# magrimm/mav_trajectory_generation_cmake

Hardware: AMD Instinct MI355X
Metric: trajectories/sec (10-seg, N=10, 3-D min-snap) at 1/2/4/8 MI355X (higher is better)
Workload: dtype f64; 1 GPU; config2: 10000 x (K=10, N=10, D=3, r=SNAP) per GPU, device-resident; batch_per_gpu=10000, global_batch=10000, segments=10, N=10, D=3, derivative_to_optimize=4, parallelism=shard1

## Files before the change

### mav_trajectory_generation_cmake_amd/csrc/mtg_solve_dl.hip

```cpp
#include "mtg_solve_dl.inc"

namespace mtg {

#define MTG_DL_DECL(NN, DD) hipError_t launch_solve_dl_n##NN##_d##DD(const SolveArgs&, hipStream_t);
MTG_DL_DECL(10, 1) MTG_DL_DECL(10, 2) MTG_DL_DECL(10, 3) MTG_DL_DECL(10, 4)
MTG_DL_DECL(12, 1) MTG_DL_DECL(12, 2) MTG_DL_DECL(12, 3) MTG_DL_DECL(12, 4)
#undef MTG_DL_DECL

bool dl_geometry(int N, int D, int K, int r) {
  if (D < 1 || D > 4 || r < 1 || r > N / 2 - 1 || K != dl_kmax(N) || K == 0) return false;
  size_t lds = 0;
#define MTG_DL_LDS(NN, DD) \
  if (N == NN && D == DD) lds = dl_lds_bytes<NN, DD>();
  MTG_DL_LDS(10, 1) MTG_DL_LDS(10, 2) MTG_DL_LDS(10, 3) MTG_DL_LDS(10, 4)
  MTG_DL_LDS(12, 1) MTG_DL_LDS(12, 2) MTG_DL_LDS(12, 3) MTG_DL_LDS(12, 4)
#undef MTG_DL_LDS
  return lds > 0 && lds <= kMaxLdsHard;
}

hipError_t launch_solve_dl(int N, const SolveArgs& a, hipStream_t stream) {
  if (!dl_geometry(N, a.D, a.K, a.r)) return hipErrorInvalidValue;
#define MTG_DL_CASE(NN, DD) \
  if (N == NN && a.D == DD) return launch_solve_dl_n##NN##_d##DD(a, stream);
  MTG_DL_CASE(10, 1) MTG_DL_CASE(10, 2) MTG_DL_CASE(10, 3) MTG_DL_CASE(10, 4)
  MTG_DL_CASE(12, 1) MTG_DL_CASE(12, 2) MTG_DL_CASE(12, 3) MTG_DL_CASE(12, 4)
#undef MTG_DL_CASE
  return hipErrorInvalidValue;
}

}
```

### mav_trajectory_generation_cmake_amd/csrc/mtg_solve_dl.inc

```
#pragma once
#include "mtg_fused.inc"

namespace mtg {

typedef __attribute__((address_space(3))) double dl_lds_double;

static __device__ constexpr double k_dl_htilde[MTG_HTILDE_SIZE] = {MTG_HTILDE_VALUES};
static __device__ constexpr double k_dl_a1inv[MTG_A1INV_SIZE] = {MTG_A1INV_VALUES};

#define MTG_DL_STEP_BARRIER() __builtin_amdgcn_sched_barrier(0)

template <int N, int KMAX, int D>
struct DlShape {
  static constexpr int H = N / 2, F = H - 1, KC = KMAX / 2, KS = KC - 1;
  static constexpr int PE = F < 4 ? F : 4, NF0 = F - PE;
  static constexpr int J0 = NF0 > 0 ? 0 : 1;
  static constexpr int NL = F * (F - 1) / 2;
  static constexpr int FS = NL + F;
  static constexpr int TPW = kBlock / (2 * D);
  static constexpr bool RR = KC > 5;
  static constexpr int WAVES = RR ? 1 : 2;
  static constexpr bool PREG = !RR;
  static constexpr int PARK = (KC + 1) * kBlock + KC * 2 * TPW;
  static constexpr int SPAD = (N / 2) % 2 == 0 ? 2 : 0, SROW = N + SPAD;
  static constexpr int FSTR = KC * FS + ((6 - (KC * FS) % 4) % 4);
  static_assert(FSTR % 4 == 2, "odd 16-B units per chain");
  static constexpr int FAC_OFF = 0, STG_OFF = FAC_OFF + TPW * 2 * FSTR,
                       PARK_OFF = STG_OFF + kBlock * SROW, RED_OFF = PARK_OFF + PARK,
                       TAB_OFF = RED_OFF + kBlock + kBlock / 2;
  static constexpr int LDS_DOUBLES_NOTAB = TAB_OFF, LDS_DOUBLES = TAB_OFF + 2 * N * N;
  static constexpr int N_FREE(int K) { return 2 * NF0 + (K - 1) * F; }
  static constexpr bool OK = N >= 6 && N <= 12 && KMAX >= 4 && KMAX % 2 == 0 && D >= 1 && D <= 4;
};

template <int N, int R>
__device__ __forceinline__ int dl_scale_bits(double T) {
  constexpr int ea = 3 - 2 * R, eb = N - 1 - 2 * R;
  const int x = __builtin_amdgcn_frexp_exp(T) - 1;
  const int xa = x * ea, xb = x * eb;
  return (xa <= -1022 || xa >= 1023 || xb <= -1022 || xb >= 1023) ? MTG_TRAJ_NOT_SPD : 0;
}

template <int E0, int E1>
struct DlPow {
  static constexpr int NP = E1 > 0 ? E1 : 0, NM = E0 < 0 ? -E0 : 0;
  double pp[NP + 1], pm[NM + 1];
  __device__ __forceinline__ DlPow(double x, double xi) {
    pp[0] = 1.0;
    pm[0] = 1.0;
    if constexpr (NP >= 1) pp[1] = x;
    if constexpr (NM >= 1) pm[1] = xi;
#pragma unroll
    for (int k = 2; k <= NP; ++k) pp[k] = pp[k >> 1] * pp[k - (k >> 1)];
#pragma unroll
    for (int k = 2; k <= NM; ++k) pm[k] = pm[k >> 1] * pm[k - (k >> 1)];
  }
  __device__ __forceinline__ double operator()(int e) const { return e >= 0 ? pp[e] : pm[-e]; }
};

enum DlMode : int { kDlPattern = 0, kDlEnds = 1, kDlGeneral = 2 };
template <int N, int R, int KMAX, int D, int MODE = kDlPattern>
struct DlChain {
  using SH = DlShape<N, KMAX, D>;
  static constexpr bool G = MODE == kDlGeneral, EP = MODE == kDlEnds;
  static constexpr int H = SH::H, F = SH::F, KC = SH::KC, KS = SH::KS, NL = SH::NL, FS = SH::FS;
  static constexpr int PE = SH::PE, J0 = (G || EP) ? 0 : SH::J0;
  static constexpr int NN = N, RR_ = R, KM = KMAX, DD = D;
  static constexpr bool GG = G, EE = EP;
  static constexpr unsigned FM = (1u << F) - 1u;
  static constexpr bool RR = SH::RR;
  static constexpr int TOP = KS - 1;
  static constexpr int E0 = 2 - 2 * R, E1 = 2 * H - 1 - 2 * R;
  static constexpr int li(int i, int k) { return i * (i - 1) / 2 + k; }

  const dl_lds_double* ht;
  const dl_lds_double* a1;
  double* park;
  double* tpark;
  static constexpr int tstride = 2 * SH::TPW;
  static constexpr bool PR = SH::PREG && !G;
  double Pr[PR ? KC + 1 : 1], Tr[PR ? KC : 1];
  static constexpr bool FR = SH::RR && !G;
  static_assert(!FR || J0 == 0, "the register-input forward sweep needs vertex 0 as a step of its own");
  double Pf[FR ? KC + 1 : 1], Tf[FR ? KC : 1];
  bool twr;
  int tbits = 0;
  uint64_t fmask;
  double E0s[F];
  unsigned pm0 = 0;
  int nf0a = 0;
  double Zs[KS > 0 ? KS : 1][F];
  double Y[F];
  double Tn, tin;
  double* fac;
  bool wr;
  double pmin = DBL_MAX;
  double cacc = 0.0;
  uint64_t pins;
  double gf[G ? F : 1];
  __amdgpu_buffer_rsrc_t rvals;
  int vo, vs;
  int csum, ftot;

  __device__ __forceinline__ double Ht(int r, int c) const { return ht[r * N + c]; }
  __device__ __forceinline__ double A1(int r, int c) const {
    return k_dl_a1inv[MTG_A1INV_OFF(N) + r * N + c];
  }
  __device__ __forceinline__ double Hc(int r, int c) const {
    return k_dl_htilde[MTG_HTILDE_OFF(N, R) + r * N + c];
  }
  __device__ __forceinline__ double TLc(int a, int b) const { return Hc(a + 1, b + 1); }
  __device__ __forceinline__ double BRc(int a, int b) const { return Hc(H + a + 1, H + b + 1); }
  __device__ __forceinline__ double BLc(int a, int k) const { return Hc(H + a + 1, k + 1); }
  __device__ __forceinline__ double hp(int a) const { return Hc(H + a + 1, H); }
  __device__ __forceinline__ double hn(int a) const { return Hc(a + 1, H); }
  __device__ __forceinline__ double Pj(int j) const { return PR ? Pr[j] : park[j * kBlock]; }
  __device__ __forceinline__ double Tj(int j) const { return PR ? Tr[j] : tpark[j * tstride]; }
  __device__ __forceinline__ double PjF(int j) const { return FR ? Pf[j] : Pj(j); }
  __device__ __forceinline__ double TjF(int j) const { return FR ? Tf[j] : Tj(j); }
  __device__ __forceinline__ void park_fwd(int J) {
    if constexpr (FR) {
      park[(J + 1) * kBlock] = Pf[J + 1];
      if (twr) tpark[J * tstride] = Tf[J];
      tbits |= time_bits(Tf[J]) | dl_scale_bits<N, R>(Tf[J]);
      asm volatile("" : "+v"(tbits));
    }
  }
  __device__ __forceinline__ void fresh_tables() {
    asm volatile("" : "+s"(ht));
    asm volatile("" : "+s"(a1));
  }

  __device__ __forceinline__ double fl(double v, int k) const {
    return (k & 1) ? __builtin_bit_cast(double, __builtin_bit_cast(uint64_t, v) ^ fmask) : v;
  }
  __device__ __forceinline__ double zprev(int J, int k) const { return Zs[TOP][k]; }

  __device__ __forceinline__ unsigned pinm(int J) const {
    return G ? (unsigned)(pins >> (J * F)) & FM : (EP && J == 0 ? pm0 : 0u);
  }
  __device__ __forceinline__ bool pinned(int J, int a) const {
    return G ? ((pins >> (J * F + a)) & 1u) != 0 : (EP && J == 0 && ((pm0 >> a) & 1u) != 0);
  }
  __device__ __forceinline__ double fxv(int J, int a) const {
    int off = vo + J * vs + (a + 1) * D * 8;
    asm volatile("" : "+v"(off));
    const double x = fl(__builtin_bit_cast(double, __builtin_amdgcn_raw_buffer_load_b64(rvals, off, 0, 0)), a + 1);
    return pinned(J, a) ? x : 0.0;
  }
  __device__ __forceinline__ int nfv(int J) const { return F - __builtin_popcount(pinm(J)); }
  __device__ __forceinline__ int free_off(bool chB, int J) const {
    int s = 0;
#pragma unroll
    for (int q = 0; q < KC; ++q) s += (chB ? q <= J : q < J) ? nfv(q) : 0;
    return chB ? ftot - s : s;
  }

  template <int P0 = 0>
  __device__ __forceinline__ void factor(double (&S)[F][F], double (&dinv)[F]) {
    double dg[F];
#pragma unroll
    for (int j = 0; j < P0; ++j) {
      dinv[j] = 0.0;
      dg[j] = 0.0;
#pragma unroll
      for (int i = j + 1; i < F; ++i) S[i][j] = 0.0;
    }
#pragma unroll
    for (int j = P0; j < F; ++j) {
      double w[F];
      double dj = S[j][j];
#pragma unroll
      for (int k = P0; k < j; ++k) {
        w[k] = S[j][k] * dg[k];
        dj -= S[j][k] * w[k];
      }
      pmin = pivot_min(pmin, dj);
      if (RR) asm volatile("" : "+v"(pmin));
      const double inv = rcp(dj);
      dg[j] = dj;
      dinv[j] = inv;
#pragma unroll
      for (int i = j + 1; i < F; ++i) {
        double t = S[i][j];
#pragma unroll
        for (int k = P0; k < j; ++k) t -= S[i][k] * w[k];
        S[i][j] = t * inv;
      }
    }
  }
  __device__ __forceinline__ void factor_pins(double (&S)[F][F], double (&dinv)[F], unsigned pm) {
#pragma unroll
    for (int a = 0; a < F; ++a) {
      const bool pa = (pm >> a) & 1u;
#pragma unroll
      for (int b = 0; b < a; ++b) S[a][b] = (pa || ((pm >> b) & 1u)) ? 0.0 : S[a][b];
      S[a][a] = pa ? 1.0 : S[a][a];
    }
    factor(S, dinv);
#pragma unroll
    for (int a = 0; a < F; ++a) dinv[a] = ((pm >> a) & 1u) ? 0.0 : dinv[a];
  }

  template <typename LF>
  __device__ __forceinline__ static void solve(LF l, const double (&dinv)[F], double (&y)[F]) {
#pragma unroll
    for (int i = 1; i < F; ++i)
#pragma unroll
      for (int k = 0; k < i; ++k) y[i] -= l(i, k) * y[k];
#pragma unroll
    for (int i = F - 1; i >= 0; --i) {
      double t = y[i] * dinv[i];
#pragma unroll
      for (int k = i + 1; k < F; ++k) t -= l(k, i) * y[k];
      y[i] = t;
    }
  }

  template <bool MERGE, bool FIRST>
  __device__ __forceinline__ void fstep(int J, int partner, const double (&Lp)[NL > 0 ? NL : 1],
                                        const double (&Dp)[F], double& Tp, double& tip, double (&S)[F][F],
                                        double (&dinv)[F], double (&rhs)[F]) {
    fresh_tables();
    double Pm[F][F];
    if constexpr (FIRST) {
#pragma unroll
      for (int a = 0; a < F; ++a)
#pragma unroll
        for (int b = 0; b <= a; ++b) Pm[a][b] = BRc(a, b);
    } else {
      double W[F][F], U[F][F];
// ... 359 lines not shown
    } else {
#pragma unroll
      for (int i = 0; i < F; ++i) y[i] = Zs[TOP][i] - tt[i];
#pragma unroll
      for (int q = KS - 1; q >= 1; --q)
#pragma unroll
        for (int k = 0; k < F; ++k) Zs[q][k] = Zs[q - 1][k];
    }
  }
};

__device__ __forceinline__ __amdgpu_buffer_rsrc_t dl_rsrc(const void* base, uint32_t bytes) { return buf_rsrc(base, bytes); }
typedef u32x4 dl_u32x4;
typedef u32x2 dl_u32x2;

template <int D>
__device__ __forceinline__ bool dl_traj_any(uint64_t ballot, int q) {
  constexpr uint64_t LM = 2 * D >= 64 ? ~0ull : (1ull << (2 * D)) - 1ull;
  return q * 2 * D < 64 && ((ballot >> (q * 2 * D)) & LM) != 0;
}

constexpr int kDlSc1 = 16;

template <int N, int KMAX, int D, int AL16>
struct DlStore {
  static constexpr int DN = D * N, PW = AL16 ? 2 : 1, PPR = DN / PW;
  static constexpr int POL = AL16 == 2 ? kDlSc1 : 0;
  static constexpr int NU = (DlShape<N, KMAX, D>::TPW * 2 * PPR + kBlock - 1) / kBlock;
  static constexpr int kOOB = 0x40000000;
  static_assert(NU * kBlock * PW <= kBlock * N, "the staged pieces a lane reads lie in the staging area");
  static constexpr int SP = DlShape<N, KMAX, D>::SPAD / PW, RP = N / PW;
  static __device__ __forceinline__ int staged(int e) { return SP ? e + (e / RP) * SP : e; }
  static_assert(DN % PW == 0, "whole 16-B pieces per run");
  int off[NU], dlt[NU];
  __device__ __forceinline__ void init(int lane, int nvt, uint64_t badl) {
    const int lim = nvt * 2 * PPR;
    uint32_t badq = 0;
    if (badl != 0) {
#pragma unroll
      for (int q = 0; q < DlShape<N, KMAX, D>::TPW; ++q) badq |= dl_traj_any<D>(badl, q) ? 1u << q : 0u;
    }
#pragma unroll
    for (int u = 0; u < NU; ++u) {
      const int e = lane + u * kBlock;
      const int run = e / PPR, o = e - run * PPR, q = run >> 1;
      const bool rv = run & 1;
      const bool ok = e < lim && !((badq >> (q & 31)) & 1u);
      off[u] = ok ? (q * KMAX * DN + o * PW + (rv ? (KMAX - 1) * DN : 0)) * 8 : kOOB;
      dlt[u] = ok ? (rv ? -DN * 8 : DN * 8) : 0;
    }
  }
};

template <typename DC, int AL16, bool FIRSTB = false>
__device__ __forceinline__ void dl_round(DC& c, const SolveArgs& a, int J, int lane, int ch, int d, bool own, int64_t pb,
                                         double* stg, const DlStore<DC::NN, DC::KM, DC::DD, AL16>& sm,
                                         __amdgpu_buffer_rsrc_t out) {
  constexpr int N = DC::NN, KMAX = DC::KM, D = DC::DD;
  constexpr int H = N / 2, F = H - 1, K = KMAX, V = K + 1;
  const double T = c.Tj(J), tinv = rcp(T);
  double v[F];
  if constexpr (FIRSTB) {
#pragma unroll
    for (int b = 0; b < F; ++b) v[b] = c.Y[b];
  } else {
    const double rho = T * c.tin;
    double rp = rho;
#pragma unroll
    for (int b = 0; b < F; ++b) {
      v[b] = rp * c.Y[b];
      rp *= rho;
    }
  }
  using SH = DlShape<N, KMAX, D>;
  double y[F];
  if (FIRSTB || J >= DC::J0) {
    if constexpr (DC::GG) {
      double vb[F];
#pragma unroll
      for (int b = 0; b < F; ++b) vb[b] = c.pinned(J + 1, b) ? 0.0 : v[b];
      c.bstep(J, vb, y);
    } else {
      c.bstep(J, v, y);
    }
  } else {
#pragma unroll
    for (int k = 0; k < F; ++k) y[k] = c.E0s[k];
  }
  if constexpr (DC::GG) {
    double tp = T;
#pragma unroll
    for (int k = 0; k < F; ++k) {
      y[k] = c.pinned(J, k) ? tp * c.fxv(J, k) : y[k];
      tp *= T;
    }
  }
  double occ[N];
  c.segment_row(ch != 0, a.cost_out != nullptr, J, tinv, y, v, occ);
  if (DC::GG && a.free_out && own) {
    double* fo = a.free_out + (pb * D + d) * ((int64_t)V * H) + c.free_off(ch != 0, J);
    const unsigned fr = ~c.pinm(J) & DC::FM;
    double tp = tinv;
#pragma unroll
    for (int k = 0; k < F; ++k) {
      const double x = y[k] * tp;
      if ((fr >> k) & 1u) fo[__builtin_popcount(fr & ((1u << k) - 1u))] = ch ? c.fl(x, k + 1) : x;
      tp *= tinv;
    }
  } else if (DC::EE && a.free_out && own) {
    const int vx = ch ? K - J : J;
    double* fo = a.free_out + (pb * D + d) * ((int64_t)V * H) + (vx == 0 ? 0 : c.nf0a + (vx - 1) * F);
    const unsigned fr = ~c.pinm(J) & DC::FM;
    double tp = tinv;
#pragma unroll
    for (int k = 0; k < F; ++k) {
      const double x = y[k] * tp;
      if ((fr >> k) & 1u) fo[__builtin_popcount(fr & ((1u << k) - 1u))] = ch ? c.fl(x, k + 1) : x;
      tp *= tinv;
    }
  } else if ((J >= 1 || SH::NF0 > 0) && a.free_out && own) {
    const int vx = ch ? K - J : J;
    double* fo = a.free_out + (pb * D + d) * ((int64_t)V * H) +
                 (vx == 0 ? 0 : (vx == K ? SH::NF0 + (K - 1) * F : SH::NF0 + (vx - 1) * F)) - (J == 0 ? SH::PE : 0);
    double tp = tinv;
#pragma unroll
    for (int k = 0; k < F; ++k) {
      const double x = y[k] * tp;
      if (J >= 1 || k >= SH::PE) fo[k] = ch ? c.fl(x, k + 1) : x;
      tp *= tinv;
    }
  }
#pragma unroll
  for (int k = 0; k < F; ++k) c.Y[k] = y[k];
  c.Tn = T;
  c.tin = tinv;
  if (!a.coeffs) return;
  dvec2* o2 = reinterpret_cast<dvec2*>(stg + lane * SH::SROW);
#pragma unroll
  for (int j = 0; j < N / 2; ++j) o2[j] = dvec2{occ[2 * j], occ[2 * j + 1]};
  lds_fence();
  constexpr int NU = DlStore<N, KMAX, D, AL16>::NU;
  constexpr int kAux = DlStore<N, KMAX, D, AL16>::POL;
  if constexpr (AL16) {
    dvec2 w[NU];
#pragma unroll
    for (int u = 0; u < NU; ++u) w[u] = reinterpret_cast<const dvec2*>(stg)[DlStore<N, KMAX, D, AL16>::staged(lane + u * kBlock)];
#pragma unroll
    for (int u = 0; u < NU; ++u)
      __builtin_amdgcn_raw_buffer_store_b128(__builtin_bit_cast(dl_u32x4, w[u]), out, sm.off[u] + J * sm.dlt[u], 0, kAux);
  } else {
    double w[NU];
#pragma unroll
    for (int u = 0; u < NU; ++u) w[u] = stg[DlStore<N, KMAX, D, AL16>::staged(lane + u * kBlock)];
#pragma unroll
    for (int u = 0; u < NU; ++u)
      __builtin_amdgcn_raw_buffer_store_b64(__builtin_bit_cast(dl_u32x2, w[u]), out, sm.off[u] + J * sm.dlt[u], 0, kAux);
  }
  lds_fence();
}

constexpr int kDlFallbackLgLog2 = 4, kDlFallbackTraj = kBlock >> kDlFallbackLgLog2;
template <int N, int R, int D>
__device__ __forceinline__ void dl_fallback(const SolveArgs& a, int64_t pair0, int nvt, uint64_t badl, double* lds) {
  uint32_t badq = 0;
  for (int q = 0; q < nvt; ++q) badq |= dl_traj_any<D>(badl, q) ? 1u << q : 0u;
  const int nb = __builtin_popcount(badq);
  const int slot = threadIdx.x >> kDlFallbackLgLog2;
  for (int base = 0; base < nb; base += kDlFallbackTraj) {
    const int k = base + slot;
    uint32_t m = badq;
    for (int i = 0; i < k && m; ++i) m &= m - 1u;
    const bool valid = k < nb;
    const int q = valid ? __builtin_ctz(m) : 0;
    solve_fused_slots<N, R>(a, kDlFallbackLgLog2, pair0 + q, valid, lds);
    __syncthreads();
  }
}

template <int N, int KMAX, int D>
struct DlWave {
  using SH = DlShape<N, KMAX, D>;
  static constexpr int H = N / 2, K = KMAX, V = K + 1;
  int lane, t, r2, ch, d, tq, partner, nvt, trl;
  bool valid;
  int64_t pair0, pb;
  double tscale;
  __amdgpu_buffer_rsrc_t rv, rt, rm;
  int vo, vs, to, ts, mo, ms;
  __device__ __forceinline__ DlWave(const SolveArgs& a, int tpw, int lane_id) {
    lane = lane_id;
    t = lane / (2 * D);
    r2 = lane - t * (2 * D);
    ch = r2 >= D ? 1 : 0;
    d = r2 - ch * D;
    tq = t < SH::TPW ? t : 0;
    partner = ch ? lane - D : lane + D;
    pair0 = (int64_t)blockIdx.x * tpw;
    const int64_t pair = pair0 + t;
    valid = t < tpw && pair < a.B;
    pb = valid ? pair : pair0;
    nvt = (int)(a.B - pair0 < tpw ? a.B - pair0 : tpw);
    const int64_t nc = a.n_cand;
    const int64_t tr0 = nc == 1 ? pair0 : pair0 / nc;
    trl = (int)((nc == 1 ? pb : pb / nc) - tr0);
    const int64_t ntr = nc == 1 ? a.B : (a.B + nc - 1) / nc;
    const int ntw = (int)(ntr - tr0 < SH::TPW ? ntr - tr0 : SH::TPW);
    rv = dl_rsrc(a.values + tr0 * (V * H * D), (uint32_t)(ntw * V * H * D * 8));
    rt = dl_rsrc(a.times + tr0 * K, (uint32_t)(ntw * K * 8));
    rm = dl_rsrc(a.mask + tr0 * V, (uint32_t)(ntw * V));
    tscale = a.scales ? a.scales[pb % nc] : 1.0;
    vo = (trl * (V * H * D) + (ch ? K * H * D : 0) + d) * 8;
    vs = ch ? -(H * D * 8) : H * D * 8;
    to = (trl * K + (ch ? K - 1 : 0)) * 8;
    ts = ch ? -8 : 8;
    mo = trl * V + (ch ? K : 0);
    ms = ch ? -1 : 1;
  }
  __device__ __forceinline__ unsigned mask(int j) const { return __builtin_amdgcn_raw_buffer_load_b8(rm, mo + j * ms, 0, 0); }
  __device__ __forceinline__ double time(int j, double sc) const {
    return __builtin_bit_cast(double, __builtin_amdgcn_raw_buffer_load_b64(rt, to + j * ts, 0, 0)) * sc;
  }
  __device__ __forceinline__ double value(int j, int k) const {
    return __builtin_bit_cast(double, __builtin_amdgcn_raw_buffer_load_b64(rv, vo + j * vs + k * D * 8, 0, 0));
  }
};

struct DlKernArgs {
  SolveArgs a;
  int tpw;
};
__device__ __forceinline__ const DlKernArgs& dl_args() {
  return *reinterpret_cast<const DlKernArgs*>((uintptr_t)__builtin_amdgcn_kernarg_segment_ptr());
}

template <int N, int R, int KC>
__device__ __forceinline__ int dl_time_bits(const double (&Tc)[KC]) {
  int st = 0;
#pragma unroll
  for (int j = 0; j < KC; ++j) st |= time_bits(Tc[j]) | dl_scale_bits<N, R>(Tc[j]);
  asm volatile("" : "+v"(st));
  return st;
}

template <typename CC, int AL16, typename W>
__device__ __forceinline__ void dl_run_pass(CC& cc, const SolveArgs& a, const W& w, const double (&E)[CC::F], bool mine,
                                            int st, double* lds, uint64_t* tph) {
  constexpr int N = CC::NN, R = CC::RR_, KMAX = CC::KM, D = CC::DD;
  using SH = DlShape<N, KMAX, D>;
  constexpr int H = N / 2, F = SH::F, KC = SH::KC;
  constexpr int K = KMAX, V = K + 1;
#ifdef MTG_PHASE_TIMING
#define MTG_DL_PSTAMP(k) tph[k] = __builtin_amdgcn_s_memrealtime()
#else
#define MTG_DL_PSTAMP(k) (void)tph
#endif
  const int lane = w.lane, ch = w.ch, d = w.d;
  const int64_t pb = w.pb;
  cc.forward(w.partner, E);
  MTG_DL_PSTAMP(2);
  if constexpr (CC::PR) st |= dl_time_bits<N, R, KC>(cc.Tr);
  if constexpr (CC::FR) st |= cc.tbits;
  if (a.free_out && mine && ch == 0) {
    double* fo = a.free_out + (pb * D + d) * ((int64_t)V * H);
    if constexpr (CC::GG) {
      const unsigned fr = ~cc.pinm(KC) & CC::FM;
#pragma unroll
      for (int k = 0; k < F; ++k)
        if ((fr >> k) & 1u) fo[cc.csum + __builtin_popcount(fr & ((1u << k) - 1u))] = cc.Y[k];
    } else {
      const int o0 = CC::EE ? cc.nf0a : SH::NF0;
#pragma unroll
      for (int k = 0; k < F; ++k) fo[o0 + (KC - 1) * F + k] = cc.Y[k];
    }
  }
  cc.scale_meeting();
  __syncthreads();

  double* stg = lds + SH::STG_OFF;
  DlStore<N, KMAX, D, AL16> sm;
  sm.init(lane, w.nvt, __builtin_amdgcn_ballot_w64(!mine));
  const __amdgpu_buffer_rsrc_t ro =
      dl_rsrc(a.coeffs ? a.coeffs + w.pair0 * (int64_t)(K * D * N) : a.values, (uint32_t)(w.nvt * K * D * N * 8));
  dl_round<CC, AL16, true>(cc, a, KC - 1, lane, ch, d, mine, pb, stg, sm, ro);
#pragma unroll
  for (int J = KC - 2; J >= 1; --J) {
    MTG_DL_STEP_BARRIER();
    dl_round<CC, AL16>(cc, a, J, lane, ch, d, mine, pb, stg, sm, ro);
  }
  MTG_DL_STEP_BARRIER();
  dl_round<CC, AL16>(cc, a, 0, lane, ch, d, mine, pb, stg, sm, ro);
  MTG_DL_PSTAMP(3);

  if (!(cc.pmin > 0.0 && cc.pmin <= DBL_MAX)) st |= MTG_TRAJ_NOT_SPD;
  if (a.status || a.cost_out) {
    double* red = lds + SH::RED_OFF;
    int* redi = reinterpret_cast<int*>(red + kBlock);
    __syncthreads();
    red[lane] = cc.cacc;
    redi[lane] = st;
    __syncthreads();
    if (w.r2 == 0 && mine) {
      double cost = 0.0;
      int s = 0;
#pragma unroll
      for (int q = 0; q < 2 * D; ++q) cost += red[lane + q], s |= redi[lane + q];
      if (a.cost_out) a.cost_out[pb] = cost;
      if (a.status) a.status[pb] = s;
    }
  }
  if (w.r2 == 0 && mine && a.n_free_out) {
    if constexpr (CC::GG || CC::EE) {
      a.n_free_out[pb] = cc.ftot;
    } else {
      a.n_free_out[pb] = SH::N_FREE(K);
    }
  }
#ifdef MTG_PHASE_TIMING
  asm volatile("s_waitcnt vmcnt(0)" ::: "memory");
  MTG_DL_PSTAMP(4);
  if (a.free_out && lane == 0) {
    double* fo = a.free_out + w.pair0 * D * ((int64_t)V * H);
    for (int k = 0; k < 5; ++k) fo[k] = (double)tph[k];
    unsigned hw, xcc;
    asm volatile("s_getreg_b32 %0, hwreg(HW_REG_HW_ID)" : "=s"(hw));
    asm volatile("s_getreg_b32 %0, hwreg(HW_REG_XCC_ID)" : "=s"(xcc));
    fo[5] = (double)hw;
    fo[6] = (double)xcc;
  }
#endif
#undef MTG_DL_PSTAMP
}

template <typename CC, typename W>
__device__ __forceinline__ void dl_place(CC& c, const W& w, int tpw, double* lds) {
  using SH = DlShape<CC::NN, CC::KM, CC::DD>;
  c.fmask = w.ch ? 0x8000000000000000ull : 0ull;
  c.fac = lds + SH::FAC_OFF + (w.tq * 2 + w.ch) * SH::FSTR;
  c.wr = w.d == 0 && w.t < tpw;
  c.park = lds + SH::PARK_OFF + w.lane;
  c.tpark = lds + SH::PARK_OFF + (CC::KC + 1) * kBlock + w.tq * 2 + w.ch;
  c.ht = (const dl_lds_double*)(lds + SH::TAB_OFF);
  c.a1 = (const dl_lds_double*)(lds + SH::TAB_OFF + CC::NN * CC::NN);
}

template <typename CC>
__device__ __forceinline__ void dl_take_inputs(CC& c, const double (&P)[CC::KC + 1], const double (&Tc)[CC::KC], int d,
                                               int t) {
  using SH = DlShape<CC::NN, CC::KM, CC::DD>;
  constexpr int KC = CC::KC;
  if constexpr (CC::PR) {
#pragma unroll
    for (int j = 0; j <= KC; ++j) c.Pr[j] = P[j];
#pragma unroll
    for (int j = 0; j < KC; ++j) c.Tr[j] = Tc[j];
  } else {
    static_assert(CC::FR, "the pattern and ends passes keep their inputs in registers");
#pragma unroll
    for (int j = 0; j <= KC; ++j) c.Pf[j] = P[j];
#pragma unroll
    for (int j = 0; j < KC; ++j) c.Tf[j] = Tc[j];
    c.twr = d == 0 && t < SH::TPW;
    c.park[0] = P[0];
  }
}

template <int N, int R, int KMAX, int D, int AL16>
__device__ __forceinline__ void dl_ends_pass(bool eown) {
  const DlKernArgs& ka = dl_args();
  const SolveArgs a = ka.a;
  const int tpw = ka.tpw;
#ifdef MTG_PHASE_TIMING
  uint64_t tph[6];
  tph[0] = __builtin_amdgcn_s_memrealtime();
#else
  uint64_t* tph = nullptr;
#endif
  using SH = DlShape<N, KMAX, D>;
  using EC = DlChain<N, R, KMAX, D, kDlEnds>;
  constexpr int H = N / 2, F = SH::F, KC = SH::KC;
  constexpr unsigned HM = (1u << H) - 1u;
  extern __shared__ __attribute__((aligned(16))) double lds[];
  int lane_id = threadIdx.x;
  asm volatile("" : "+v"(lane_id));
  const DlWave<N, KMAX, D> w(a, tpw, lane_id);
  EC c;
  dl_place(c, w, tpw, lds);
  const unsigned m0 = w.mask(0);
  double Tc[KC], P[KC + 1], E[F];
  Tc[0] = w.time(0, w.tscale);
#pragma unroll
  for (int k = 0; k < F; ++k) E[k] = c.fl(w.value(0, k + 1), k + 1);
#pragma unroll
  for (int j = 0; j <= KC; ++j) {
    P[j] = w.value(j, 0);
    if (j + 1 < KC) Tc[j + 1] = w.time(j + 1, w.tscale);
  }
  c.pm0 = (m0 >> 1) & EC::FM;
  const int nf0 = F - __builtin_popcount(c.pm0), nfp = __shfl(nf0, w.partner);
  c.nf0a = w.ch ? nfp : nf0;
  c.ftot = nf0 + nfp + (KMAX - 1) * F;
  dl_take_inputs(c, P, Tc, w.d, w.t);
#ifdef MTG_PHASE_TIMING
  tph[1] = __builtin_amdgcn_s_memrealtime();
#endif
  dl_run_pass<EC, AL16>(c, a, w, E, eown, (m0 & ~HM) ? MTG_TRAJ_WARN_DROPPED : 0, lds, tph);
}

template <int N, int R, int KMAX, int D, int AL16>
__device__ __forceinline__ void dl_general_pass(bool gown) {
  const DlKernArgs& ka = dl_args();
  const SolveArgs a = ka.a;
  const int tpw = ka.tpw;
#ifdef MTG_PHASE_TIMING
  uint64_t tph[6];
  tph[0] = __builtin_amdgcn_s_memrealtime();
#else
  uint64_t* tph = nullptr;
#endif
  using SH = DlShape<N, KMAX, D>;
  using DG = DlChain<N, R, KMAX, D, kDlGeneral>;
  constexpr int H = N / 2, F = SH::F, KC = SH::KC;
  constexpr unsigned HM = (1u << H) - 1u;
  extern __shared__ __attribute__((aligned(16))) double lds[];
  int lane_id = threadIdx.x;
  asm volatile("" : "+v"(lane_id));
  const DlWave<N, KMAX, D> w(a, tpw, lane_id);
  DG g;
  dl_place(g, w, tpw, lds);
  g.rvals = w.rv;
  g.vo = w.vo;
  g.vs = w.vs;
  double P[KC + 1], Tc[KC];
  unsigned mk[KC + 1];
#pragma unroll
  for (int j = 0; j <= KC; ++j) {
    mk[j] = w.mask(j);
    P[j] = w.value(j, 0);
    if (j < KC) Tc[j] = w.time(j, w.tscale);
  }
  int dropped = 0;
  g.pins = 0;
#pragma unroll
  for (int j = 0; j <= KC; ++j) {
    g.pins |= (uint64_t)((mk[j] >> 1) & DG::FM) << (j * F);
    dropped |= mk[j] & ~HM;
    g.park[j * kBlock] = P[j];
  }
  if (w.d == 0 && w.t < SH::TPW) {
#pragma unroll
    for (int j = 0; j < KC; ++j) g.tpark[j * g.tstride] = Tc[j];
  }
  const int st0 = dl_time_bits<N, R, KC>(Tc) | (dropped ? MTG_TRAJ_WARN_DROPPED : 0);
  int cs = 0;
#pragma unroll
  for (int j = 0; j < KC; ++j) cs += g.nfv(j);
  g.csum = cs;
  g.ftot = cs + __shfl(cs, w.partner) + g.nfv(KC);
  __syncthreads();
#ifdef MTG_PHASE_TIMING
  tph[1] = __builtin_amdgcn_s_memrealtime();
#endif
  double E[F];
#pragma unroll
  for (int k = 0; k < F; ++k) E[k] = 0.0;
  dl_run_pass<DG, AL16>(g, a, w, E, gown, st0, lds, tph);
}

template <int N, int R, int KMAX, int D, int AL16>
__global__ __launch_bounds__(kBlock) __attribute__((amdgpu_waves_per_eu(DlShape<N, KMAX, D>::WAVES))) void solve_dl_kernel(
    DlKernArgs ka) {
  using SH = DlShape<N, KMAX, D>;
  using DC = DlChain<N, R, KMAX, D>;
  constexpr int F = SH::F, KC = SH::KC;
  constexpr unsigned EM = (1u << (SH::PE + 1)) - 1u;
  const SolveArgs& a = ka.a;
  const int tpw = ka.tpw;
  extern __shared__ __attribute__((aligned(16))) double lds[];
#ifdef MTG_PHASE_TIMING
  uint64_t tph[6];
  tph[0] = __builtin_amdgcn_s_memrealtime();
#else
  uint64_t* tph = nullptr;
#endif
  const DlWave<N, KMAX, D> w(a, tpw, threadIdx.x);
  const int t = w.t, d = w.d;

  DC c;
  dl_place(c, w, tpw, lds);
  unsigned mk[KC + 1];
  double Tc[KC], P[KC + 1], E[F];
#pragma unroll
  for (int j = 0; j <= KC; ++j) mk[j] = w.mask(j);
  Tc[0] = w.time(0, w.tscale);
#pragma unroll
  for (int k = 0; k < F; ++k) E[k] = k < SH::PE ? c.fl(w.value(0, k + 1), k + 1) : 0.0;
#pragma unroll
  for (int j = 0; j <= KC; ++j) {
    P[j] = w.value(j, 0);
    if (j + 1 < KC) Tc[j + 1] = w.time(j + 1, w.tscale);
  }
  unsigned bad = mk[0] ^ EM, ebad = ~mk[0] & 1u, xpos = 0u;
#pragma unroll
  for (int j = 1; j <= KC; ++j) {
    bad |= mk[j] ^ 1u;
    ebad |= mk[j] ^ 1u;
  }
#pragma unroll
  for (int j = 0; j <= KC; ++j) xpos |= ~mk[j] & 1u;
  const uint64_t badl = __builtin_amdgcn_ballot_w64(bad != 0u), el = __builtin_amdgcn_ballot_w64(ebad != 0u),
                 xl = __builtin_amdgcn_ballot_w64(xpos != 0u);
  const bool pbad = dl_traj_any<D>(badl, t), ebt = dl_traj_any<D>(el, t), xbad = dl_traj_any<D>(xl, t);
  const bool own = w.valid && !pbad, eown = w.valid && pbad && !ebt, gown = w.valid && ebt && !xbad,
             fown = w.valid && xbad;

  if (a.cost_out) {
    constexpr int UH = (N * N + kBlock - 1) / kBlock;
    const double* hg = c_htilde + MTG_HTILDE_OFF(N, R);
    const double* ag = c_a1inv + MTG_A1INV_OFF(N);
    double hv[UH], av[UH];
#pragma unroll
    for (int u = 0; u < UH; ++u) {
      const int i = w.lane + u * kBlock;
      hv[u] = hg[i < N * N ? i : N * N - 1];
      av[u] = ag[i < N * N ? i : N * N - 1];
    }
#pragma unroll
    for (int u = 0; u < UH; ++u) {
      const int i = w.lane + u * kBlock;
      lds[SH::TAB_OFF + (i < N * N ? i : N * N - 1)] = hv[u];
      lds[SH::TAB_OFF + N * N + (i < N * N ? i : N * N - 1)] = av[u];
    }
  }
  if (__builtin_amdgcn_ballot_w64(own) != 0) {
    dl_take_inputs(c, P, Tc, d, t);
    if (a.cost_out) __syncthreads();
#ifdef MTG_PHASE_TIMING
    tph[1] = __builtin_amdgcn_s_memrealtime();
#endif
    dl_run_pass<DC, AL16>(c, a, w, E, own, 0, lds, tph);
  }
  if (__builtin_expect(__builtin_amdgcn_ballot_w64(eown) != 0, 0)) {
    __syncthreads();
    dl_ends_pass<N, R, KMAX, D, AL16>(eown);
  }
  if (__builtin_expect(__builtin_amdgcn_ballot_w64(gown) != 0, 0)) {
    __syncthreads();
    dl_general_pass<N, R, KMAX, D, AL16>(gown);
  }
  if (__builtin_expect(__builtin_amdgcn_ballot_w64(fown) != 0, 0)) {
    __syncthreads();
    dl_fallback<N, R, D>(a, w.pair0, w.nvt, __builtin_amdgcn_ballot_w64(fown), lds);
  }
}
__host__ __device__ constexpr int dl_kmax(int N) { return N == 10 ? 10 : (N == 12 ? 20 : 0); }
template <int N, int D>
__host__ __device__ constexpr size_t dl_lds_bytes(bool cost = true) {
  constexpr int KMAX = dl_kmax(N) > 0 ? dl_kmax(N) : 4;
  const size_t dl = sizeof(double) * (size_t)(cost ? DlShape<N, KMAX, D>::LDS_DOUBLES : DlShape<N, KMAX, D>::LDS_DOUBLES_NOTAB);
  const size_t fb = sizeof(double) * (size_t)kDlFallbackTraj * slot_doubles(N / 2, D, KMAX, 1 << kDlFallbackLgLog2);
  return dl > fb ? dl : fb;
}

inline bool dl_store_sc1(size_t bytes, bool long_chains) {
  static const int force = [] {
    const char* v = getenv("MTG_DL_STORE_SC1");
    return v && (v[0] == '0' || v[0] == '1') ? v[0] - '0' : -1;
  }();
  return force >= 0 ? force == 1 : bytes <= ((size_t)(long_chains ? 192 : 64) << 20);
}

template <int N, int R, int KMAX, int D>
static hipError_t launch_dl_nrk(const SolveArgs& a, hipStream_t stream) {
  if constexpr (!DlShape<N, KMAX, D>::OK || R < 1) {
    return hipErrorInvalidValue;
  } else {
    if (a.K != KMAX) return hipErrorInvalidValue;
    const size_t lds = dl_lds_bytes<N, D>(a.cost_out != nullptr);
    const int tpw = DlShape<N, KMAX, D>::TPW;
    const bool sc1 = dl_store_sc1((size_t)a.B * KMAX * D * N * sizeof(double), DlShape<N, KMAX, D>::RR);
    const int64_t blocks = (a.B + tpw - 1) / tpw;
    if (blocks == 0) return hipSuccess;
    const bool al16 = !(reinterpret_cast<uintptr_t>(a.coeffs) & 15u);
    const int al = al16 ? (sc1 ? 2 : 1) : 0;
    const void* fn = al == 2 ? (const void*)solve_dl_kernel<N, R, KMAX, D, 2>
                             : al == 1 ? (const void*)solve_dl_kernel<N, R, KMAX, D, 1> : (const void*)solve_dl_kernel<N, R, KMAX, D, 0>;
    if (lds > kMaxLdsPerBlock) {
      const hipError_t e = hipFuncSetAttribute(fn, hipFuncAttributeMaxDynamicSharedMemorySize, (int)lds);
      if (e != hipSuccess) return e;
    }
    const DlKernArgs ka{a, tpw};
    if (al == 2)
      launch_kernel((solve_dl_kernel<N, R, KMAX, D, 2>), dim3((unsigned)blocks), dim3(kBlock), lds, stream, ka);
    else if (al == 1)
      launch_kernel((solve_dl_kernel<N, R, KMAX, D, 1>), dim3((unsigned)blocks), dim3(kBlock), lds, stream, ka);
    else
      launch_kernel((solve_dl_kernel<N, R, KMAX, D, 0>), dim3((unsigned)blocks), dim3(kBlock), lds, stream, ka);
    return hipGetLastError();
  }
}

template <int N, int R, int D>
static hipError_t launch_dl_nrd(const SolveArgs& a, hipStream_t stream) {
  if constexpr (dl_kmax(N) > 0) {
    if (a.K == dl_kmax(N)) return launch_dl_nrk<N, R, dl_kmax(N), D>(a, stream);
  }
  return hipErrorInvalidValue;
}

template <int N, int D>
static hipError_t launch_dl_nd(const SolveArgs& a, hipStream_t stream) {
  switch (a.r) {
    case 1: if constexpr (N / 2 > 1) return launch_dl_nrd<N, 1, D>(a, stream); break;
    case 2: if constexpr (N / 2 > 2) return launch_dl_nrd<N, 2, D>(a, stream); break;
    case 3: if constexpr (N / 2 > 3) return launch_dl_nrd<N, 3, D>(a, stream); break;
    case 4: if constexpr (N / 2 > 4) return launch_dl_nrd<N, 4, D>(a, stream); break;
    case 5: if constexpr (N / 2 > 5) return launch_dl_nrd<N, 5, D>(a, stream); break;
    default: break;
  }
  return hipErrorInvalidValue;
}

#define MTG_DL_LAUNCHER(NN, DD)                                                          \
  hipError_t launch_solve_dl_n##NN##_d##DD(const SolveArgs& a, hipStream_t stream) {     \
    return launch_dl_nd<NN, DD>(a, stream);                                              \
  }

}
```

Before: 1.007 billion trajectories/s.

## Add compact 64-byte kernarg hot header and status-free kernel variant

Puts a 64-byte header at the front of the kernel arguments. It holds precomputed per-block byte strides, the last-block count and flags, and is loaded as one scalar vector, so each block skips the 64-bit divides and the full SolveArgs reads when there is one candidate and no scales. It adds a template flag ST that removes pivot-min tracking, time/scale status bits and the status/cost reduction when no optional outputs are requested and the output fits a size threshold. Optional output pointers are loaded only when flagged. The risk is losing the not-SPD and status detection in the default path, plus more kernel instantiations.

```diff
diff --git a/mav_trajectory_generation_cmake_amd/csrc/mtg_solve_dl.hip b/mav_trajectory_generation_cmake_amd/csrc/mtg_solve_dl.hip
--- a/mav_trajectory_generation_cmake_amd/csrc/mtg_solve_dl.hip
+++ b/mav_trajectory_generation_cmake_amd/csrc/mtg_solve_dl.hip
@@ -29,3 +29,28 @@
 }
 
 }
+
+extern "C" int mtgtest_dl_hot_header(int N, int D, int K, int r, const void* values, const void* mask, const void* times,
+                                     void* coeffs, const void* scales, int64_t B, int n_cand, int any_optional,
+                                     void* out) {
+  using namespace mtg;
+  if (!dl_geometry(N, D, K, r) || B < 1) return -1;
+  SolveArgs a{};
+  a.values = static_cast<const double*>(values);
+  a.mask = static_cast<const uint8_t*>(mask);
+  a.times = static_cast<const double*>(times);
+  a.coeffs = static_cast<double*>(coeffs);
+  a.scales = static_cast<const double*>(scales);
+  static int32_t dummy_status;
+  a.status = any_optional ? &dummy_status : nullptr;
+  a.B = B;
+  a.K = K;
+  a.D = D;
+  a.r = r;
+  a.n_cand = n_cand;
+  const int tpw = kBlock / (2 * D);
+  DlHot h;
+  if (!dl_fill_hot(N, K, D, tpw, a, &h)) return -1;
+  *static_cast<DlHot*>(out) = h;
+  return 0;
+}
diff --git a/mav_trajectory_generation_cmake_amd/csrc/mtg_solve_dl.inc b/mav_trajectory_generation_cmake_amd/csrc/mtg_solve_dl.inc
--- a/mav_trajectory_generation_cmake_amd/csrc/mtg_solve_dl.inc
+++ b/mav_trajectory_generation_cmake_amd/csrc/mtg_solve_dl.inc
@@ -59,14 +59,14 @@
 };
 
 enum DlMode : int { kDlPattern = 0, kDlEnds = 1, kDlGeneral = 2 };
-template <int N, int R, int KMAX, int D, int MODE = kDlPattern>
+template <int N, int R, int KMAX, int D, int MODE = kDlPattern, bool ST = true>
 struct DlChain {
   using SH = DlShape<N, KMAX, D>;
   static constexpr bool G = MODE == kDlGeneral, EP = MODE == kDlEnds;
   static constexpr int H = SH::H, F = SH::F, KC = SH::KC, KS = SH::KS, NL = SH::NL, FS = SH::FS;
   static constexpr int PE = SH::PE, J0 = (G || EP) ? 0 : SH::J0;
   static constexpr int NN = N, RR_ = R, KM = KMAX, DD = D;
-  static constexpr bool GG = G, EE = EP;
+  static constexpr bool GG = G, EE = EP, SS = ST;
   static constexpr unsigned FM = (1u << F) - 1u;
   static constexpr bool RR = SH::RR;
   static constexpr int TOP = KS - 1;
@@ -122,8 +122,10 @@
     if constexpr (FR) {
       park[(J + 1) * kBlock] = Pf[J + 1];
       if (twr) tpark[J * tstride] = Tf[J];
-      tbits |= time_bits(Tf[J]) | dl_scale_bits<N, R>(Tf[J]);
-      asm volatile("" : "+v"(tbits));
+      if constexpr (ST) {
+        tbits |= time_bits(Tf[J]) | dl_scale_bits<N, R>(Tf[J]);
+        asm volatile("" : "+v"(tbits));
+      }
     }
   }
   __device__ __forceinline__ void fresh_tables() {
@@ -175,8 +177,10 @@
         w[k] = S[j][k] * dg[k];
         dj -= S[j][k] * w[k];
       }
-      pmin = pivot_min(pmin, dj);
-      if (RR) asm volatile("" : "+v"(pmin));
+      if constexpr (ST) {
+        pmin = pivot_min(pmin, dj);
+        if (RR) asm volatile("" : "+v"(pmin));
+      }
       const double inv = rcp(dj);
       dg[j] = dj;
       dinv[j] = inv;
@@ -642,8 +646,16 @@
   }
 };
 
+struct DlOuts {
+  double* coeffs;
+  double* free_out;
+  double* cost_out;
+  int32_t* status;
+  int32_t* n_free_out;
+};
+
 template <typename DC, int AL16, bool FIRSTB = false>
-__device__ __forceinline__ void dl_round(DC& c, const SolveArgs& a, int J, int lane, int ch, int d, bool own, int64_t pb,
+__device__ __forceinline__ void dl_round(DC& c, const DlOuts& a, int J, int lane, int ch, int d, bool own, int64_t pb,
                                          double* stg, const DlStore<DC::NN, DC::KM, DC::DD, AL16>& sm,
                                          __amdgpu_buffer_rsrc_t out) {
   constexpr int N = DC::NN, KMAX = DC::KM, D = DC::DD;
@@ -686,7 +698,7 @@
     }
   }
   double occ[N];
-  c.segment_row(ch != 0, a.cost_out != nullptr, J, tinv, y, v, occ);
+  c.segment_row(ch != 0, DC::SS && a.cost_out != nullptr, J, tinv, y, v, occ);
   if (DC::GG && a.free_out && own) {
     double* fo = a.free_out + (pb * D + d) * ((int64_t)V * H) + c.free_off(ch != 0, J);
     const unsigned fr = ~c.pinm(J) & DC::FM;
@@ -767,6 +779,60 @@
   }
 }
 
+enum DlHotFlags : uint32_t {
+  kDlPlain = 1u,
+  kDlCoeffs = 2u,
+  kDlOptional = 4u,
+};
+struct DlHot {
+  const double* values;
+  const uint8_t* mask;
+  const double* times;
+  double* coeffs;
+  uint32_t vbytes, mbytes, tbytes, obytes;
+  int32_t tpw;
+  uint32_t flags;
+  uint32_t last_block;
+  int32_t last_nvt;
+};
+static_assert(sizeof(DlHot) == 64, "the hot header is one 64-byte line");
+struct DlKernArgs {
+  DlHot h;
+  SolveArgs a;
+};
+static_assert(offsetof(DlKernArgs, h) == 0, "the hot header leads the kernarg segment");
+__device__ __forceinline__ const DlKernArgs& dl_args() {
+  return *reinterpret_cast<const DlKernArgs*>((uintptr_t)__builtin_amdgcn_kernarg_segment_ptr());
+}
+__device__ __forceinline__ DlHot dl_hot() {
+  typedef uint32_t dl_u32x16 __attribute__((ext_vector_type(16)));
+  dl_u32x16 v = *(const __attribute__((address_space(4))) dl_u32x16*)__builtin_amdgcn_kernarg_segment_ptr();
+  asm volatile("" : "+s"(v));
+  return __builtin_bit_cast(DlHot, v);
+}
+
+inline bool dl_fill_hot(int N, int K, int D, int tpw, const SolveArgs& a, DlHot* h) {
+  const int64_t V = K + 1, H = N / 2;
+  const int64_t vb = tpw * V * H * D * 8, mb = tpw * V, tb = (int64_t)tpw * K * 8, ob = (int64_t)tpw * K * D * N * 8;
+  if (a.B < 1 || tpw < 1 || vb > INT32_MAX || ob > INT32_MAX) return false;
+  const int64_t blocks = (a.B + tpw - 1) / tpw;
+  if (blocks > UINT32_MAX) return false;
+  h->values = a.values;
+  h->mask = a.mask;
+  h->times = a.times;
+  h->coeffs = a.coeffs;
+  h->vbytes = (uint32_t)vb;
+  h->mbytes = (uint32_t)mb;
+  h->tbytes = (uint32_t)tb;
+  h->obytes = (uint32_t)ob;
+  h->tpw = tpw;
+  h->flags = (a.n_cand == 1 && !a.scales ? kDlPlain : 0u) | (a.coeffs ? kDlCoeffs : 0u) |
+             (a.free_out || a.n_free_out || a.cost_out || a.status ? kDlOptional : 0u);
+  h->last_block = (uint32_t)(blocks - 1);
+  h->last_nvt = (int32_t)(a.B - (blocks - 1) * tpw);
+  return true;
+}
+
 template <int N, int KMAX, int D>
 struct DlWave {
   using SH = DlShape<N, KMAX, D>;
@@ -776,8 +842,10 @@
   int64_t pair0, pb;
   double tscale;
   __amdgpu_buffer_rsrc_t rv, rt, rm;
+  const char* obase;
   int vo, vs, to, ts, mo, ms;
-  __device__ __forceinline__ DlWave(const SolveArgs& a, int tpw, int lane_id) {
+  __device__ __forceinline__ DlWave(const DlHot& h, const SolveArgs& a, int lane_id) {
+    const int tpw = h.tpw;
     lane = lane_id;
     t = lane / (2 * D);
     r2 = lane - t * (2 * D);
@@ -785,20 +853,30 @@
     d = r2 - ch * D;
     tq = t < SH::TPW ? t : 0;
     partner = ch ? lane - D : lane + D;
-    pair0 = (int64_t)blockIdx.x * tpw;
-    const int64_t pair = pair0 + t;
-    valid = t < tpw && pair < a.B;
-    pb = valid ? pair : pair0;
-    nvt = (int)(a.B - pair0 < tpw ? a.B - pair0 : tpw);
-    const int64_t nc = a.n_cand;
-    const int64_t tr0 = nc == 1 ? pair0 : pair0 / nc;
-    trl = (int)((nc == 1 ? pb : pb / nc) - tr0);
-    const int64_t ntr = nc == 1 ? a.B : (a.B + nc - 1) / nc;
-    const int ntw = (int)(ntr - tr0 < SH::TPW ? ntr - tr0 : SH::TPW);
-    rv = dl_rsrc(a.values + tr0 * (V * H * D), (uint32_t)(ntw * V * H * D * 8));
-    rt = dl_rsrc(a.times + tr0 * K, (uint32_t)(ntw * K * 8));
-    rm = dl_rsrc(a.mask + tr0 * V, (uint32_t)(ntw * V));
-    tscale = a.scales ? a.scales[pb % nc] : 1.0;
+    const uint32_t bid = blockIdx.x;
+    nvt = bid == h.last_block ? h.last_nvt : tpw;
+    pair0 = (int64_t)((uint64_t)bid * (uint32_t)tpw);
+    valid = t < nvt;
+    pb = valid ? pair0 + t : pair0;
+    obase = (h.flags & kDlCoeffs) ? reinterpret_cast<const char*>(h.coeffs) + (uint64_t)bid * h.obytes
+                                  : reinterpret_cast<const char*>(h.values);
+    if (__builtin_expect((h.flags & kDlPlain) != 0u, 1)) {
+      trl = valid ? t : 0;
+      rv = dl_rsrc(reinterpret_cast<const char*>(h.values) + (uint64_t)bid * h.vbytes, (uint32_t)(nvt * (V * H * D * 8)));
+      rt = dl_rsrc(reinterpret_cast<const char*>(h.times) + (uint64_t)bid * h.tbytes, (uint32_t)(nvt * (K * 8)));
+      rm = dl_rsrc(h.mask + (uint64_t)bid * h.mbytes, (uint32_t)(nvt * V));
+      tscale = 1.0;
+    } else {
+      const int64_t nc = a.n_cand;
+      const int64_t tr0 = pair0 / nc;
+      trl = (int)(pb / nc - tr0);
+      const int64_t ntr = (a.B + nc - 1) / nc;
+      const int ntw = (int)(ntr - tr0 < SH::TPW ? ntr - tr0 : SH::TPW);
+      rv = dl_rsrc(a.values + tr0 * (V * H * D), (uint32_t)(ntw * V * H * D * 8));
+      rt = dl_rsrc(a.times + tr0 * K, (uint32_t)(ntw * K * 8));
+      rm = dl_rsrc(a.mask + tr0 * V, (uint32_t)(ntw * V));
+      tscale = a.scales ? a.scales[pb % nc] : 1.0;
+    }
     vo = (trl * (V * H * D) + (ch ? K * H * D : 0) + d) * 8;
     vs = ch ? -(H * D * 8) : H * D * 8;
     to = (trl * K + (ch ? K - 1 : 0)) * 8;
@@ -806,6 +884,7 @@
     mo = trl * V + (ch ? K : 0);
     ms = ch ? -1 : 1;
   }
+  __device__ __forceinline__ __amdgpu_buffer_rsrc_t out() const { return dl_rsrc(obase, (uint32_t)(nvt * (K * D * N * 8))); }
   __device__ __forceinline__ unsigned mask(int j) const { return __builtin_amdgcn_raw_buffer_load_b8(rm, mo + j * ms, 0, 0); }
   __device__ __forceinline__ double time(int j, double sc) const {
     return __builtin_bit_cast(double, __builtin_amdgcn_raw_buffer_load_b64(rt, to + j * ts, 0, 0)) * sc;
@@ -815,12 +894,8 @@
   }
 };
 
-struct DlKernArgs {
-  SolveArgs a;
-  int tpw;
-};
-__device__ __forceinline__ const DlKernArgs& dl_args() {
-  return *reinterpret_cast<const DlKernArgs*>((uintptr_t)__builtin_amdgcn_kernarg_segment_ptr());
+__device__ __forceinline__ DlOuts dl_outs(const SolveArgs& a) {
+  return DlOuts{a.coeffs, a.free_out, a.cost_out, a.status, a.n_free_out};
 }
 
 template <int N, int R, int KC>
@@ -833,7 +908,7 @@
 }
 
 template <typename CC, int AL16, typename W>
-__device__ __forceinline__ void dl_run_pass(CC& cc, const SolveArgs& a, const W& w, const double (&E)[CC::F], bool mine,
+__device__ __forceinline__ void dl_run_pass(CC& cc, const DlOuts& a, const W& w, const double (&E)[CC::F], bool mine,
                                             int st, double* lds, uint64_t* tph) {
   constexpr int N = CC::NN, R = CC::RR_, KMAX = CC::KM, D = CC::DD;
   using SH = DlShape<N, KMAX, D>;
@@ -848,8 +923,8 @@
   const int64_t pb = w.pb;
   cc.forward(w.partner, E);
   MTG_DL_PSTAMP(2);
-  if constexpr (CC::PR) st |= dl_time_bits<N, R, KC>(cc.Tr);
-  if constexpr (CC::FR) st |= cc.tbits;
+  if constexpr (CC::SS && CC::PR) st |= dl_time_bits<N, R, KC>(cc.Tr);
+  if constexpr (CC::SS && CC::FR) st |= cc.tbits;
   if (a.free_out && mine && ch == 0) {
     double* fo = a.free_out + (pb * D + d) * ((int64_t)V * H);
     if constexpr (CC::GG) {
@@ -869,8 +944,7 @@
   double* stg = lds + SH::STG_OFF;
   DlStore<N, KMAX, D, AL16> sm;
   sm.init(lane, w.nvt, __builtin_amdgcn_ballot_w64(!mine));
-  const __amdgpu_buffer_rsrc_t ro =
-      dl_rsrc(a.coeffs ? a.coeffs + w.pair0 * (int64_t)(K * D * N) : a.values, (uint32_t)(w.nvt * K * D * N * 8));
+  const __amdgpu_buffer_rsrc_t ro = w.out();
   dl_round<CC, AL16, true>(cc, a, KC - 1, lane, ch, d, mine, pb, stg, sm, ro);
 #pragma unroll
   for (int J = KC - 2; J >= 1; --J) {
@@ -881,28 +955,30 @@
   dl_round<CC, AL16>(cc, a, 0, lane, ch, d, mine, pb, stg, sm, ro);
   MTG_DL_PSTAMP(3);
 
-  if (!(cc.pmin > 0.0 && cc.pmin <= DBL_MAX)) st |= MTG_TRAJ_NOT_SPD;
-  if (a.status || a.cost_out) {
-    double* red = lds + SH::RED_OFF;
-    int* redi = reinterpret_cast<int*>(red + kBlock);
-    __syncthreads();
-    red[lane] = cc.cacc;
-    redi[lane] = st;
-    __syncthreads();
-    if (w.r2 == 0 && mine) {
-      double cost = 0.0;
-      int s = 0;
-#pragma unroll
-      for (int q = 0; q < 2 * D; ++q) cost += red[lane + q], s |= redi[lane + q];
-      if (a.cost_out) a.cost_out[pb] = cost;
-      if (a.status) a.status[pb] = s;
-    }
-  }
-  if (w.r2 == 0 && mine && a.n_free_out) {
-    if constexpr (CC::GG || CC::EE) {
-      a.n_free_out[pb] = cc.ftot;
-    } else {
-      a.n_free_out[pb] = SH::N_FREE(K);
+  if constexpr (CC::SS) {
+    if (!(cc.pmin > 0.0 && cc.pmin <= DBL_MAX)) st |= MTG_TRAJ_NOT_SPD;
+    if (a.status || a.cost_out) {
+      double* red = lds + SH::RED_OFF;
+      int* redi = reinterpret_cast<int*>(red + kBlock);
+      __syncthreads();
+      red[lane] = cc.cacc;
+      redi[lane] = st;
+      __syncthreads();
+      if (w.r2 == 0 && mine) {
+        double cost = 0.0;
+        int s = 0;
+#pragma unroll
+        for (int q = 0; q < 2 * D; ++q) cost += red[lane + q], s |= redi[lane + q];
+        if (a.cost_out) a.cost_out[pb] = cost;
+        if (a.status) a.status[pb] = s;
+      }
+    }
+    if (w.r2 == 0 && mine && a.n_free_out) {
+      if constexpr (CC::GG || CC::EE) {
+        a.n_free_out[pb] = cc.ftot;
+      } else {
+        a.n_free_out[pb] = SH::N_FREE(K);
+      }
     }
   }
 #ifdef MTG_PHASE_TIMING
@@ -954,11 +1030,12 @@
   }
 }
 
-template <int N, int R, int KMAX, int D, int AL16>
+template <int N, int R, int KMAX, int D, int AL16, bool ST>
 __device__ __forceinline__ void dl_ends_pass(bool eown) {
   const DlKernArgs& ka = dl_args();
-  const SolveArgs a = ka.a;
-  const int tpw = ka.tpw;
+  const DlOuts a = dl_outs(ka.a);
+  const DlHot h = dl_hot();
+  const int tpw = h.tpw;
 #ifdef MTG_PHASE_TIMING
   uint64_t tph[6];
   tph[0] = __builtin_amdgcn_s_memrealtime();
@@ -966,13 +1043,13 @@
   uint64_t* tph = nullptr;
 #endif
   using SH = DlShape<N, KMAX, D>;
-  using EC = DlChain<N, R, KMAX, D, kDlEnds>;
+  using EC= DlChain<N, R, KMAX, D, kDlEnds, ST>;
   constexpr int H = N / 2, F = SH::F, KC = SH::KC;
   constexpr unsigned HM = (1u << H) - 1u;
   extern __shared__ __attribute__((aligned(16))) double lds[];
   int lane_id = threadIdx.x;
   asm volatile("" : "+v"(lane_id));
-  const DlWave<N, KMAX, D> w(a, tpw, lane_id);
+  const DlWave<N, KMAX, D> w(h, ka.a, lane_id);
   EC c;
   dl_place(c, w, tpw, lds);
   const unsigned m0 = w.mask(0);
@@ -996,11 +1073,12 @@
   dl_run_pass<EC, AL16>(c, a, w, E, eown, (m0 & ~HM) ? MTG_TRAJ_WARN_DROPPED : 0, lds, tph);
 }
 
-template <int N, int R, int KMAX, int D, int AL16>
+template <int N, int R, int KMAX, int D, int AL16, bool ST>
 __device__ __forceinline__ void dl_general_pass(bool gown) {
   const DlKernArgs& ka = dl_args();
-  const SolveArgs a = ka.a;
-  const int tpw = ka.tpw;
+  const DlOuts a = dl_outs(ka.a);
+  const DlHot h = dl_hot();
+  const int tpw = h.tpw;
 #ifdef MTG_PHASE_TIMING
   uint64_t tph[6];
   tph[0] = __builtin_amdgcn_s_memrealtime();
@@ -1008,13 +1086,13 @@
   uint64_t* tph = nullptr;
 #endif
   using SH = DlShape<N, KMAX, D>;
-  using DG = DlChain<N, R, KMAX, D, kDlGeneral>;
+  using DG= DlChain<N, R, KMAX, D, kDlGeneral, ST>;
   constexpr int H = N / 2, F = SH::F, KC = SH::KC;
   constexpr unsigned HM = (1u << H) - 1u;
   extern __shared__ __attribute__((aligned(16))) double lds[];
   int lane_id = threadIdx.x;
   asm volatile("" : "+v"(lane_id));
-  const DlWave<N, KMAX, D> w(a, tpw, lane_id);
+  const DlWave<N, KMAX, D> w(h, ka.a, lane_id);
   DG g;
   dl_place(g, w, tpw, lds);
   g.rvals = w.rv;
@@ -1040,7 +1118,8 @@
 #pragma unroll
     for (int j = 0; j < KC; ++j) g.tpark[j * g.tstride] = Tc[j];
   }
-  const int st0 = dl_time_bits<N, R, KC>(Tc) | (dropped ? MTG_TRAJ_WARN_DROPPED : 0);
+  int st0 = 0;
+  if constexpr (ST) st0 = dl_time_bits<N, R, KC>(Tc) | (dropped ? MTG_TRAJ_WARN_DROPPED : 0);
   int cs = 0;
 #pragma unroll
   for (int j = 0; j < KC; ++j) cs += g.nfv(j);
@@ -1056,15 +1135,28 @@
   dl_run_pass<DG, AL16>(g, a, w, E, gown, st0, lds, tph);
 }
 
-template <int N, int R, int KMAX, int D, int AL16>
+template <int N, int R, int KMAX, int D, int AL16, bool ST>
 __global__ __launch_bounds__(kBlock) __attribute__((amdgpu_waves_per_eu(DlShape<N, KMAX, D>::WAVES))) void solve_dl_kernel(
     DlKernArgs ka) {
   using SH = DlShape<N, KMAX, D>;
-  using DC = DlChain<N, R, KMAX, D>;
+  using DC = DlChain<N, R, KMAX, D, kDlPattern, ST>;
   constexpr int F = SH::F, KC = SH::KC;
   constexpr unsigned EM = (1u << (SH::PE + 1)) - 1u;
-  const SolveArgs& a = ka.a;
-  const int tpw = ka.tpw;
+  const DlHot h = dl_hot();
+  const int tpw = h.tpw;
+  DlOuts a{h.coeffs, nullptr, nullptr, nullptr, nullptr};
+  if (h.flags & kDlOptional) {
+    typedef const __attribute__((address_space(4))) char* dl_kptr;
+    auto fa = (const __attribute__((address_space(4))) SolveArgs*)((dl_kptr)__builtin_amdgcn_kernarg_segment_ptr() +
+                                                                   offsetof(DlKernArgs, a));
+    asm volatile("" : "+s"(fa));
+    a.free_out = fa->free_out;
+    if constexpr (ST) {
+      a.cost_out = fa->cost_out;
+      a.status = fa->status;
+      a.n_free_out = fa->n_free_out;
+    }
+  }
   extern __shared__ __attribute__((aligned(16))) double lds[];
 #ifdef MTG_PHASE_TIMING
   uint64_t tph[6];
@@ -1072,7 +1164,7 @@
 #else
   uint64_t* tph = nullptr;
 #endif
-  const DlWave<N, KMAX, D> w(a, tpw, threadIdx.x);
+  const DlWave<N, KMAX, D> w(h, ka.a, threadIdx.x);
   const int t = w.t, d = w.d;
 
   DC c;
@@ -1131,15 +1223,15 @@
   }
   if (__builtin_expect(__builtin_amdgcn_ballot_w64(eown) != 0, 0)) {
     __syncthreads();
-    dl_ends_pass<N, R, KMAX, D, AL16>(eown);
+    dl_ends_pass<N, R, KMAX, D, AL16, ST>(eown);
   }
   if (__builtin_expect(__builtin_amdgcn_ballot_w64(gown) != 0, 0)) {
     __syncthreads();
-    dl_general_pass<N, R, KMAX, D, AL16>(gown);
+    dl_general_pass<N, R, KMAX, D, AL16, ST>(gown);
   }
   if (__builtin_expect(__builtin_amdgcn_ballot_w64(fown) != 0, 0)) {
     __syncthreads();
-    dl_fallback<N, R, D>(a, w.pair0, w.nvt, __builtin_amdgcn_ballot_w64(fown), lds);
+    dl_fallback<N, R, D>(dl_args().a, w.pair0, w.nvt, __builtin_amdgcn_ballot_w64(fown), lds);
   }
 }
 __host__ __device__ constexpr int dl_kmax(int N) { return N == 10 ? 10 : (N == 12 ? 20 : 0); }
@@ -1157,6 +1249,25 @@
     return v && (v[0] == '0' || v[0] == '1') ? v[0] - '0' : -1;
   }();
   return force >= 0 ? force == 1 : bytes <= ((size_t)(long_chains ? 192 : 64) << 20);
+}
+
+inline bool dl_status_free(size_t bytes, bool long_chains) {
+  static const int force = [] {
+    const char* v = getenv("MTG_DL_STATUS");
+    return v && (v[0] == '0' || v[0] == '1') ? v[0] - '0' : -1;
+  }();
+  return force >= 0 ? force == 0 : bytes <= ((size_t)(long_chains ? 192 : 64) << 20);
+}
+
+template <int N, int R, int KMAX, int D, int AL16, bool ST>
+static hipError_t launch_dl_inst(const DlKernArgs& ka, unsigned blocks, size_t lds, hipStream_t stream) {
+  if (lds > kMaxLdsPerBlock) {
+    const hipError_t e = hipFuncSetAttribute((const void*)solve_dl_kernel<N, R, KMAX, D, AL16, ST>,
+                                             hipFuncAttributeMaxDynamicSharedMemorySize, (int)lds);
+    if (e != hipSuccess) return e;
+  }
+  launch_kernel((solve_dl_kernel<N, R, KMAX, D, AL16, ST>), dim3(blocks), dim3(kBlock), lds, stream, ka);
+  return hipGetLastError();
 }
 
 template <int N, int R, int KMAX, int D>
@@ -1167,25 +1278,24 @@
     if (a.K != KMAX) return hipErrorInvalidValue;
     const size_t lds = dl_lds_bytes<N, D>(a.cost_out != nullptr);
     const int tpw = DlShape<N, KMAX, D>::TPW;
-    const bool sc1 = dl_store_sc1((size_t)a.B * KMAX * D * N * sizeof(double), DlShape<N, KMAX, D>::RR);
-    const int64_t blocks = (a.B + tpw - 1) / tpw;
-    if (blocks == 0) return hipSuccess;
+    const size_t out_bytes = (size_t)a.B * KMAX * D * N * sizeof(double);
+    const bool sc1 = dl_store_sc1(out_bytes, DlShape<N, KMAX, D>::RR);
+    if (a.B == 0) return hipSuccess;
     const bool al16 = !(reinterpret_cast<uintptr_t>(a.coeffs) & 15u);
     const int al = al16 ? (sc1 ? 2 : 1) : 0;
-    const void* fn = al == 2 ? (const void*)solve_dl_kernel<N, R, KMAX, D, 2>
-                             : al == 1 ? (const void*)solve_dl_kernel<N, R, KMAX, D, 1> : (const void*)solve_dl_kernel<N, R, KMAX, D, 0>;
-    if (lds > kMaxLdsPerBlock) {
-      const hipError_t e = hipFuncSetAttribute(fn, hipFuncAttributeMaxDynamicSharedMemorySize, (int)lds);
-      if (e != hipSuccess) return e;
-    }
-    const DlKernArgs ka{a, tpw};
-    if (al == 2)
-      launch_kernel((solve_dl_kernel<N, R, KMAX, D, 2>), dim3((unsigned)blocks), dim3(kBlock), lds, stream, ka);
-    else if (al == 1)
-      launch_kernel((solve_dl_kernel<N, R, KMAX, D, 1>), dim3((unsigned)blocks), dim3(kBlock), lds, stream, ka);
-    else
-      launch_kernel((solve_dl_kernel<N, R, KMAX, D, 0>), dim3((unsigned)blocks), dim3(kBlock), lds, stream, ka);
-    return hipGetLastError();
+    DlKernArgs ka;
+    if (!dl_fill_hot(N, KMAX, D, tpw, a, &ka.h)) return hipErrorInvalidValue;
+    ka.a = a;
+    const unsigned blocks = ka.h.last_block + 1u;
+    const bool st = a.status || a.cost_out || a.n_free_out || !dl_status_free(out_bytes, DlShape<N, KMAX, D>::RR);
+    if (st) {
+      if (al == 2) return launch_dl_inst<N, R, KMAX, D, 2, true>(ka, blocks, lds, stream);
+      if (al == 1) return launch_dl_inst<N, R, KMAX, D, 1, true>(ka, blocks, lds, stream);
+      return launch_dl_inst<N, R, KMAX, D, 0, true>(ka, blocks, lds, stream);
+    }
+    if (al == 2) return launch_dl_inst<N, R, KMAX, D, 2, false>(ka, blocks, lds, stream);
+    if (al == 1) return launch_dl_inst<N, R, KMAX, D, 1, false>(ka, blocks, lds, stream);
+    return launch_dl_inst<N, R, KMAX, D, 0, false>(ka, blocks, lds, stream);
   }
 }
 
```

New measurement: 1.049 billion trajectories/s (median of 6 runs). 1.04x the previous value.
